# ArtoriasAbyssslayer/HashModNFFBanks-IDR

Measured on AMD Instinct MI355X. Metric: rays/sec fwd+bwd (hash+SDF MLP), higher is better.
Workload: dtype f32; 1 GPU; DTU-shaped synthetic uniform-sphere rays, MultiResHash L=16 T=2^19 F=2 (BASELINE.json configs[1]), full IDR training step (forward + IDRLoss + backward + clip + Adam), weights held at the geometric initialisation (lr = 0): the SURVEY.md 8(d) workload; grid_config=C2, rays_per_gpu=2048, global_rays=2048, parallelism=single GPU, world=1, ranks_seen=1, step=HIP-graph captured static-shape step

## Files before the change

hashmodnffbanks_idr_amd/csrc/hm_sdf.hip:

```cpp
#include "hm_common.h"

#include <math.h>
#include <stdlib.h>

namespace {

#include "hm_sdf_common.h"
#include "hm_trace_dev.h"

#ifdef HM_SDF_PHASE_PROBE
__device__ unsigned long long hm_probe_ts[128];
#define HM_PROBE(i_)                                                                                  \
    do {                                                                                              \
        if (blockIdx.x == 0 && threadIdx.x == 0 && it == 1 && (i_) < 120) hm_probe_ts[(i_)] = wall_clock64(); \
        if (blockIdx.x == 0 && threadIdx.x == 0 && it == 1 && ((i_) == 0 || (i_) == 100))                 \
            hm_probe_ts[120 + ((i_) != 0)] = clock64();         \
    } while (0)
#define HM_PROBE_WAVES(base_)                                                                                  \
    do {                                                                                                       \
        if (blockIdx.x == 0 && (threadIdx.x & 63) == 0 && it == 1 && li == 2) hm_probe_ts[(base_) + (threadIdx.x >> 6)] = wall_clock64(); \
    } while (0)
#define HM_PROBE_S(i_)                                                                                \
    do {                                                                                              \
        if (blockIdx.x == 0 && threadIdx.x == 0 && (i_) < 120) hm_probe_ts[(i_)] = wall_clock64();   \
// ... 361 lines not shown
        else if (n_loc <= 8 && !body16)
            sdf_small_body<FRAC, Tile8<8>>(lv, net, xp, n_loc, table, Bf, vp, 1, 1, lds, 0, 1 << 30);
        else
            sdf_small_body<FRAC, Tile16>(lv, net, xp, n_loc, table, Bf, vp, 1, 1, lds, 0, 1 << 30);
        __syncthreads();
        if (tid == 0) ctl[0] = 0;
        __syncthreads();
        if (mine) march_advance_ray(a, ray, ctl, slot_base);
        __syncthreads();
    }
}

__global__ __launch_bounds__(kThreadsSdf, 2) void mfma_f32_stream_kernel(int iters, float *out) {
    f32x16 acc00 = {0}, acc01 = {0}, acc10 = {0}, acc11 = {0};
    float a0 = (float)(threadIdx.x & 63) * 1e-3f, a1 = a0 + 0.5f, b0 = 1.0f - a0, b1 = 0.25f + a0;
    for (int it = 0; it < iters; ++it) {
#pragma unroll
        for (int r = 0; r < 4; ++r) {
            acc00 = __builtin_amdgcn_mfma_f32_32x32x2f32(a0, b0, acc00, 0, 0, 0);
            acc01 = __builtin_amdgcn_mfma_f32_32x32x2f32(a0, b1, acc01, 0, 0, 0);
            acc10 = __builtin_amdgcn_mfma_f32_32x32x2f32(a1, b0, acc10, 0, 0, 0);
            acc11 = __builtin_amdgcn_mfma_f32_32x32x2f32(a1, b1, acc11, 0, 0, 0);
        }
    }
    out[(size_t)blockIdx.x * kThreadsSdf + threadIdx.x] = acc00[0] + acc01[5] + acc10[9] + acc11[15];
}

__device__ __attribute__((noinline)) void secant_step_ray(const TraceArgs &a, int64_t q, int last) {
    secant_advance_ray(a, q, last);
}

template <int FRAC>
__device__ __forceinline__ void secant_role(const HmLevels &lv, const SdfNet &net, const float *__restrict__ table,
                                            const float *__restrict__ Bf, const TraceArgs &a, int n_iters, int64_t n,
                                            int pts, float *lds) {
    const int64_t n_tiles = (n + pts - 1) / pts;
    for (int it = 0; it < n_iters; ++it) {
        if (pts == 4)
            sdf_small_body<FRAC, Tile8<4>>(lv, net, a.w.pts, n, table, Bf, a.w.vals, 1, 1, lds, blockIdx.x, gridDim.x);
        else if (pts == 8)
            sdf_small_body<FRAC, Tile8<8>>(lv, net, a.w.pts, n, table, Bf, a.w.vals, 1, 1, lds, blockIdx.x, gridDim.x);
        else
            sdf_small_body<FRAC, Tile16>(lv, net, a.w.pts, n, table, Bf, a.w.vals, 1, 1, lds, blockIdx.x, gridDim.x);
        __syncthreads();
        for (int64_t tile = blockIdx.x; tile < n_tiles; tile += gridDim.x) {
            const int64_t q = tile * pts + threadIdx.x;
            if ((int)threadIdx.x < pts && q < n) secant_step_ray(a, q, it == n_iters - 1 ? 1 : 0);
        }
        __syncthreads();
    }
}

template <int FRAC>
__global__ __launch_bounds__(kThreadsSdf, 1) void trace_secant_kernel(HmLevels lv, SdfNet net,
                                                                       const float *__restrict__ table,
                                                                       const float *__restrict__ Bf, TraceArgs a,
                                                                       int n_iters, int64_t m8_max, int64_t m4_max,
                                                                       int64_t scan_hide) {
    extern __shared__ __align__(16) float lds[];
    const int64_t n = a.w.cnt[C_NSEC];
    if (n <= 0) return;
    const bool as_scan = scan_hide > 0 && a.w.cnt[C_NSEL_PTS] >= scan_hide;
    const int pts = as_scan ? 16 : (n <= m4_max ? 4 : (n <= m8_max ? 8 : 16));
    secant_role<FRAC>(lv, net, table, Bf, a, n_iters, n, pts, lds);
}

template <int FRAC>
__global__ __launch_bounds__(kThreadsSdf, 2) void sdf_scan_secant_kernel(HmLevels lv, SdfNet net,
                                                                          const float *__restrict__ table,
                                                                          const float *__restrict__ Bf, TraceArgs a,
                                                                          int n_iters, int64_t m8_max, int64_t m4_max,
                                                                          const float *__restrict__ scan_x,
                                                                          float *__restrict__ scan_out, int c_scan,
                                                                          int64_t scan_cap, int64_t scan_min,
                                                                          int64_t scan_hide, int c_prev1, int grid1,
                                                                          int c_prev2, int grid2) {
    extern __shared__ __align__(16) float lds[];
    const int64_t n_scan = min((int64_t)max(a.w.cnt[c_scan], 0), scan_cap);
    const int64_t n_sec = a.w.cnt[C_NSEC];
    if (n_sec > 0 && n_iters > 0) {
        const int pts = a.w.cnt[C_NSEL_PTS] >= scan_hide ? 16 : (n_sec <= m4_max ? 4 : (n_sec <= m8_max ? 8 : 16));
        secant_role<FRAC>(lv, net, table, Bf, a, n_iters, n_sec, pts, lds);
    }
    if (n_scan < scan_min) return;
    const int64_t tb = (n_scan + kPts - 1) / kPts;
    int64_t done = c_prev1 >= 0 ? fill_quota(max(a.w.cnt[c_prev1], 0), grid1, tb, scan_min) : 0;
    if (c_prev2 >= 0) done += fill_quota(max(a.w.cnt[c_prev2], 0), grid2, tb - done, scan_min);
    const int64_t skip = done * kPts;
    if (skip >= n_scan) return;
    const SdfFill none = {nullptr, nullptr, 0, 0};
    sdf64_run<FRAC, true>(lv, net, scan_x + skip * 3, n_scan - skip, table, Bf, scan_out + skip, 1, 1, lds,
                          reinterpret_cast<unsigned *>(a.w.cnt + C_TILE_CURSOR), none);
}

template <int KIND, int FRAC>
__device__ __forceinline__ void split_scan_range(const HmLevels &lv, const SdfNet &net_split, const float *__restrict__ table,
                                                 const float *__restrict__ Bf, const TraceArgs &a, int64_t scan_off,
                                                 int64_t n_scan, int64_t first, int64_t quota, unsigned *cursor, float *lds) {
    __shared__ unsigned s_scan_tile;
    if (quota <= 0) return;
    for (;;) {
        __syncthreads();
        if (threadIdx.x == 0) s_scan_tile = atomicAdd(cursor, 1u);
        __syncthreads();
        const int64_t k = s_scan_tile;
        if (k >= quota) break;
        sdf_split_tile<KIND, FRAC>(lv, net_split, a.w.pts + scan_off * 3, n_scan, table, Bf, a.w.vals + scan_off, 1, lds,
                                   first + k);
    }
}

template <int KIND, int FRAC>
__global__ __launch_bounds__(kThreadsSdf, 2) void sdf_refine_scan_kernel(HmLevels lv, SdfNet net, SdfNet net_split,
                                                                          const float *__restrict__ table,
                                                                          const float *__restrict__ Bf, TraceArgs a,
                                                                          int c_ref1, int c_ref2, int which,
                                                                          int64_t scan_off, int64_t chain_tiles) {
    extern __shared__ __align__(16) float lds[];
    const int64_t n_ref1 = min((int64_t)max(a.w.cnt[c_ref1], 0), a.w.cap);
    const int64_t n_ref2 = which ? min((int64_t)max(a.w.cnt[c_ref2], 0), a.w.cap) : 0;
    const int64_t n_ref = which ? n_ref2 : n_ref1;
    const int64_t n_scan = min((int64_t)max(a.w.cnt[C_NSEL_PTS], 0), a.w.cap);
    if (n_ref > 0) {
        const SdfFill none = {nullptr, nullptr, 0, 0};
        sdf64_run<FRAC, true>(lv, net, a.w.ref_pts, n_ref, table, Bf, a.w.ref_vals, 1, 1, lds,
                              reinterpret_cast<unsigned *>(a.w.cnt + (which ? C_XREF2_CURSOR : C_XREF_CURSOR)), none);
    }
    const ScanPool p = scan_pool_quota(n_scan, n_ref1, n_ref2, c_ref2 >= 0, gridDim.x, a.w.cnt[C_NSAMP], chain_tiles);
    split_scan_range<KIND, FRAC>(lv, net_split, table, Bf, a, scan_off, n_scan, which ? p.first[1] : p.first[0],
                                 which ? p.quota[1] : p.quota[0],
                                 reinterpret_cast<unsigned *>(a.w.cnt + (which ? C_XSCAN2_CURSOR : C_XSCAN_CURSOR)), lds);
}

template <int KIND, int FRAC>
__global__ __launch_bounds__(kThreadsSdf, 2) void sdf_split_scan_secant_kernel(HmLevels lv, SdfNet net, SdfNet net_split,
                                                                                const float *__restrict__ table,
                                                                                const float *__restrict__ Bf, TraceArgs a,
                                                                                int n_iters, int64_t m8_max, int64_t m4_max,
                                                                                int64_t scan_hide, int c_ref1, int c_ref2,
                                                                                int grid_x, int64_t scan_off,
                                                                                int64_t chain_tiles) {
    extern __shared__ __align__(16) float lds[];
    const int64_t n_sec = a.w.cnt[C_NSEC];
    if (n_sec > 0 && n_iters > 0) {
        const int pts = a.w.cnt[C_NSEL_PTS] >= scan_hide ? 16 : (n_sec <= m4_max ? 4 : (n_sec <= m8_max ? 8 : 16));
        secant_role<FRAC>(lv, net, table, Bf, a, n_iters, n_sec, pts, lds);
    }
    const int64_t n_scan = min((int64_t)max(a.w.cnt[C_NSEL_PTS], 0), a.w.cap);
    const int64_t n_ref1 = min((int64_t)max(a.w.cnt[c_ref1], 0), a.w.cap);
    const int64_t n_ref2 = c_ref2 >= 0 ? min((int64_t)max(a.w.cnt[c_ref2], 0), a.w.cap) : 0;
    const ScanPool p = scan_pool_quota(n_scan, n_ref1, n_ref2, c_ref2 >= 0, grid_x, a.w.cnt[C_NSAMP], chain_tiles);
    split_scan_range<KIND, FRAC>(lv, net_split, table, Bf, a, scan_off, n_scan, p.first[2], p.quota[2],
                                 reinterpret_cast<unsigned *>(a.w.cnt + C_YSCAN_CURSOR), lds);
}

static int sdf_net_fp32(const char *who, const HmLevels &lv, const hm_mlp_desc *mlp, int64_t emb_stride, SdfImage img,
                        SdfNet &net, bool *all_m16 = nullptr) {
    return sdf_net_from_desc(who, mlp, lv.E, emb_stride, img, 1, (lv.E + 7) / 8 * 2, false, net, all_m16);
}

constexpr size_t kLds16Max = 96 * 1024, kLds64Max = 160 * 1024, kLdsTrace = 64;

static int sdf_fp32_fits(const hm_mlp_desc *mlp, int E) {
    HmLevels lv = {};
    lv.E = E;
    SdfNet net;
    bool have16 = true;
    const int rc = sdf_net_fp32("hm_sdf_net_fits", lv, mlp, 0, kImgM16Optional, net, &have16);
    if (rc != HM_OK) return rc;
    HM_CHECK_ARG(sdf_lds64(net).bytes() + kLdsTrace <= kLds64Max, "hm_sdf_net_fits: network does not fit the 160 KB LDS tile");
    HM_CHECK_ARG(!have16 || sdf_lds_small(net, E, kPts16).bytes() + kLdsTrace <= kLds16Max,
                 "hm_sdf_net_fits: network does not fit the 16-point LDS tile");
    return HM_OK;
}

struct SmallTiles {
    int64_t m8_max, m4_max;
};
static SmallTiles sdf_small_tiles(int tile_points) {
// ... 100 lines not shown
        HM_CHECK_LAUNCH("hm_trace_march_tail");
        return HM_OK;
    });
}

int hm_trace_secant_persistent(const hm_grid_desc *desc, const hm_mlp_desc *mlp, const float *table, const float *B_fourier,
                               int frac_mode, int tile_points, const void *trace_args, int n_iters, int scan_rule,
                               void *stream) {
    HM_CHECK_ARG(desc && mlp && table && B_fourier && trace_args, "hm_trace_secant_persistent: NULL argument");
    HM_CHECK_ARG(frac_mode == HM_FRAC_REFERENCE || frac_mode == HM_FRAC_TRILINEAR, "hm_trace_secant_persistent: bad frac_mode");
    HM_CHECK_ARG(tile_points == 0 || tile_points == 4 || tile_points == 8 || tile_points == 16,
                 "hm_trace_secant_persistent: tile_points must be 0, 4, 8 or 16");
    const TraceArgs &a = *static_cast<const TraceArgs *>(trace_args);
    SdfNet net;
    const int rc = sdf_net_fp32("hm_trace_secant_persistent", desc->lv, mlp, 0, kImgM16, net);
    if (rc != HM_OK) return rc;
    if (a.n == 0 || n_iters <= 0) return HM_OK;
    const size_t lds = sdf_lds_small(net, desc->lv.E, kPts16).bytes();
    HM_CHECK_ARG(lds <= kLds16Max, "hm_trace_secant_persistent: network does not fit the 16-point LDS tile");
    const SmallTiles t = sdf_small_tiles(tile_points);
    const unsigned grid = sdf_small_grid(a.n, t, 256);
    return hm_frac_dispatch(frac_mode, [&](auto frac) {
        constexpr auto kernel = trace_secant_kernel<decltype(frac)::value>;
        const int rc = hm_allow_dynamic_lds<kernel>(96 * 1024);
        if (rc != HM_OK) return rc;
        hipLaunchKernelGGL(kernel, dim3(grid), dim3(kThreadsSdf), lds, as_stream(stream), desc->lv, net, table, B_fourier,
                           a, n_iters, t.m8_max, t.m4_max, (int64_t)((scan_rule && tile_points == 0) ? kTraceScanHide : 0));
        HM_CHECK_LAUNCH("hm_trace_secant_persistent");
        return HM_OK;
    });
}

int hm_trace_scan_secant(const hm_grid_desc *desc, const hm_mlp_desc *mlp, const float *table, const float *B_fourier,
                         int frac_mode, const void *trace_args, int n_iters, const float *scan_x, float *scan_out,
                         int64_t scan_capacity, int c_scan, int small_front, int c_prev1, int grid1, int c_prev2, int grid2,
                         void *stream) {
    HM_CHECK_ARG(desc && mlp && table && B_fourier && trace_args, "hm_trace_scan_secant: NULL argument");
    HM_CHECK_ARG(frac_mode == HM_FRAC_REFERENCE || frac_mode == HM_FRAC_TRILINEAR, "hm_trace_scan_secant: bad frac_mode");
    HM_CHECK_ARG(c_scan >= 0 && c_scan < C_COUNT && scan_capacity >= 0, "hm_trace_scan_secant: bad scan counter / capacity");
    HM_CHECK_ARG(small_front || (grid1 <= 0 && grid2 <= 0), "hm_trace_scan_secant: a refinement list has no filler tiles");
    const TraceArgs &a = *static_cast<const TraceArgs *>(trace_args);
    SdfNet net;
    int rc = sdf_net_fp32("hm_trace_scan_secant", desc->lv, mlp, 0, kImgM16, net);
    if (rc != HM_OK) return rc;
    if (a.n == 0) return HM_OK;
    HM_CHECK_ARG(scan_x && scan_out, "hm_trace_scan_secant: NULL scan pointer");
    if (small_front) {
        rc = hm_sdf_fwd(desc, mlp, scan_x, scan_capacity, table, B_fourier, scan_out, 1, 1, frac_mode, -1, a.w.cnt + c_scan, 0,
                        stream);
        if (rc != HM_OK) return rc;
    }
    const size_t lds16 = sdf_lds_small(net, desc->lv.E, kPts16).bytes(), lds64 = sdf_lds64(net).bytes();
    HM_CHECK_ARG(lds16 <= kLds16Max && lds64 <= kLds64Max - kLdsTrace, "hm_trace_scan_secant: network does not fit the LDS tiles");
    const size_t lds = lds16 > lds64 ? lds16 : lds64;
    static_assert(kTraceScanHide == 3 * 256 * kPts, "kTraceScanHide counts rounds of 64-point tiles");
    const int64_t scan_hide = kTraceScanHide;
    const int p1 = grid1 > 0 ? c_prev1 : -1, p2 = grid2 > 0 ? c_prev2 : -1;
    const SmallTiles t = sdf_small_tiles(0);
    return hm_frac_dispatch(frac_mode, [&](auto frac) {
        constexpr auto kernel = sdf_scan_secant_kernel<decltype(frac)::value>;
        const int rc = hm_allow_dynamic_lds<kernel>(160 * 1024 - 64);
        if (rc != HM_OK) return rc;
        hipLaunchKernelGGL(kernel, dim3(256), dim3(kThreadsSdf), lds, as_stream(stream), desc->lv, net, table, B_fourier, a,
                           n_iters, t.m8_max, t.m4_max, scan_x, scan_out, c_scan, scan_capacity,
                           (int64_t)(small_front ? kSdfSmall + 1 : 1), scan_hide, p1, grid1, p2, grid2);
        HM_CHECK_LAUNCH("hm_trace_scan_secant");
        return HM_OK;
    });
}

int hm_trace_refine_scan(const hm_grid_desc *desc, const hm_mlp_desc *mlp, const float *table, const float *B_fourier,
                         int frac_mode, const void *trace_args, int c_ref1, int c_ref2, int which, int64_t scan_off,
                         int64_t scan_capacity, int64_t chain_tiles, void *stream) {
    HM_CHECK_ARG(desc && mlp && table && B_fourier && trace_args, "hm_trace_refine_scan: NULL argument");
    HM_CHECK_ARG(frac_mode == HM_FRAC_REFERENCE || frac_mode == HM_FRAC_TRILINEAR, "hm_trace_refine_scan: bad frac_mode");
    HM_CHECK_ARG(c_ref1 >= 0 && c_ref1 < C_COUNT && c_ref2 < C_COUNT, "hm_trace_refine_scan: bad list counter");
    HM_CHECK_ARG((which == 0 || which == 1) && (which == 0 || c_ref2 >= 0) && chain_tiles >= 0,
                 "hm_trace_refine_scan: bad launch index / chain capacity");
    const TraceArgs &a = *static_cast<const TraceArgs *>(trace_args);
    static_assert(sizeof(HmLevels) + 2 * sizeof(SdfNet) + sizeof(TraceArgs) + 64 <= 4096, "kernel arguments exceed 4 KB");
    SdfNet net, net_split;
    size_t lds_split = 0;
    int rc = sdf_net_fp32("hm_trace_refine_scan", desc->lv, mlp, 0, kImgM16, net);
    if (rc == HM_OK) rc = sdf_split_net("hm_trace_refine_scan", desc->lv.E, mlp, 0, net_split, &lds_split);
    if (rc != HM_OK) return rc;
    if (a.n == 0) return HM_OK;
    HM_CHECK_ARG(a.w.pts && a.w.vals && a.w.ref_pts && a.w.ref_vals && a.w.cnt, "hm_trace_refine_scan: NULL workspace pointer");
    HM_CHECK_ARG(scan_off >= 0 && scan_capacity >= 0 && scan_capacity <= a.w.cap, "hm_trace_refine_scan: bad scan region");
    if (which == 0) {
        rc = hm_sdf_fwd(desc, mlp, a.w.pts + scan_off * 3, scan_capacity, table, B_fourier, a.w.vals + scan_off, 1, 1,
                        frac_mode, -1, a.w.cnt + C_NSEL_PTS, 0, stream);
        if (rc != HM_OK) return rc;
    }
    const size_t lds64 = sdf_lds64(net).bytes();
    HM_CHECK_ARG(lds64 <= kLds64Max - kLdsTrace && lds_split <= kLds64Max - kLdsTrace,
                 "hm_trace_refine_scan: network does not fit the LDS tiles");
    const size_t lds = lds_split > lds64 ? lds_split : lds64;
    const unsigned grid = refine_scan_grid(a.w.cap);
    const auto launch = [&](auto kind, auto frac) {
        constexpr auto kernel = sdf_refine_scan_kernel<decltype(kind)::value, decltype(frac)::value>;
        const int rc = hm_allow_dynamic_lds<kernel>(160 * 1024 - 64);
        if (rc != HM_OK) return rc;
        hipLaunchKernelGGL(kernel, dim3(grid), dim3(kThreadsSdf), lds, as_stream(stream), desc->lv, net, net_split, table,
                           B_fourier, a, c_ref1, c_ref2, which, scan_off, chain_tiles);
        HM_CHECK_LAUNCH("hm_trace_refine_scan");
        return HM_OK;
    };
    return hm_frac_dispatch(frac_mode, [&](auto frac) {
        if (mlp->split_kind == HM_SPLIT_BF16X2) return launch(std::integral_constant<int, HM_SPLIT_BF16X2>{}, frac);
        return launch(std::integral_constant<int, HM_SPLIT_F16X2>{}, frac);
    });
}

int hm_trace_split_scan_secant(const hm_grid_desc *desc, const hm_mlp_desc *mlp, const float *table,
                               const float *B_fourier, int frac_mode, const void *trace_args, int n_iters, int c_ref1,
                               int c_ref2, int64_t scan_off, int64_t scan_capacity, int64_t chain_tiles, void *stream) {
    HM_CHECK_ARG(desc && mlp && table && B_fourier && trace_args, "hm_trace_split_scan_secant: NULL argument");
    HM_CHECK_ARG(frac_mode == HM_FRAC_REFERENCE || frac_mode == HM_FRAC_TRILINEAR,
                 "hm_trace_split_scan_secant: bad frac_mode");
    HM_CHECK_ARG(c_ref1 >= 0 && c_ref1 < C_COUNT && c_ref2 < C_COUNT && chain_tiles >= 0,
                 "hm_trace_split_scan_secant: bad list counter / chain capacity");
    const TraceArgs &a = *static_cast<const TraceArgs *>(trace_args);
    SdfNet net, net_split;
    size_t lds_split = 0;
    int rc = sdf_net_fp32("hm_trace_split_scan_secant", desc->lv, mlp, 0, kImgM16, net);
    if (rc == HM_OK) rc = sdf_split_net("hm_trace_split_scan_secant", desc->lv.E, mlp, 0, net_split, &lds_split);
    if (rc != HM_OK) return rc;
    if (a.n == 0) return HM_OK;
    HM_CHECK_ARG(a.w.pts && a.w.vals && a.w.cnt, "hm_trace_split_scan_secant: NULL workspace pointer");
    HM_CHECK_ARG(scan_off >= 0 && scan_capacity >= 0 && scan_capacity <= a.w.cap, "hm_trace_split_scan_secant: bad scan region");
    const size_t lds16 = sdf_lds_small(net, desc->lv.E, kPts16).bytes();
    HM_CHECK_ARG(lds16 <= kLds16Max && lds_split <= kLds64Max - kLdsTrace,
                 "hm_trace_split_scan_secant: network does not fit the LDS tiles");
    const size_t lds = lds16 > lds_split ? lds16 : lds_split;
    const int grid_x = (int)refine_scan_grid(a.w.cap);
    const SmallTiles t = sdf_small_tiles(0);
    const auto launch = [&](auto kind, auto frac) {
        constexpr auto kernel = sdf_split_scan_secant_kernel<decltype(kind)::value, decltype(frac)::value>;
        const int rc = hm_allow_dynamic_lds<kernel>(160 * 1024 - 64);
        if (rc != HM_OK) return rc;
        hipLaunchKernelGGL(kernel, dim3(256), dim3(kThreadsSdf), lds, as_stream(stream), desc->lv, net, net_split, table,
                           B_fourier, a, n_iters, t.m8_max, t.m4_max, (int64_t)kTraceScanHide, c_ref1, c_ref2, grid_x,
                           scan_off, chain_tiles);
        HM_CHECK_LAUNCH("hm_trace_split_scan_secant");
        return HM_OK;
    };
    return hm_frac_dispatch(frac_mode, [&](auto frac) {
        if (mlp->split_kind == HM_SPLIT_BF16X2) return launch(std::integral_constant<int, HM_SPLIT_BF16X2>{}, frac);
        return launch(std::integral_constant<int, HM_SPLIT_F16X2>{}, frac);
    });
}

int hm_trace_scan_pool_plan(int64_t n_scan, int64_t n_ref1, int64_t n_ref2, int two_x, int grid_x, int64_t n_sec_bound,
                            int n_iters, int64_t chain_tiles, int64_t *first, int64_t *quota) {
    HM_CHECK_ARG(n_scan >= 0 && n_ref1 >= 0 && n_ref2 >= 0 && grid_x >= 1 && grid_x <= 256 && n_sec_bound >= 0 &&
                     n_iters >= 0 && chain_tiles >= -1 && first && quota,
                 "hm_trace_scan_pool_plan: bad argument");
    const ScanPool p = scan_pool_quota(n_scan, n_ref1, n_ref2, two_x != 0, grid_x, n_sec_bound,
                                       trace_chain_tiles(n_iters, chain_tiles));
    for (int k = 0; k < 3; ++k) {
        first[k] = p.first[k];
        quota[k] = p.quota[k];
    }
    return HM_OK;
}

static int sdf_fwd_impl(const HmLevels &lv, const hm_mlp_desc *mlp, const float *x, int64_t emb_stride, int64_t n,
                        const float *table, const float *B_fourier, float *out, int64_t out_stride, int out_cols,
                        int frac_mode, int tile_points, const int32_t *n_dev, int max_workgroups, void *stream,
                        const SdfFillArgs *fill, int *grid64_out) {
    HM_CHECK_ARG(n >= 0, "hm_sdf_fwd: n < 0");
    HM_CHECK_ARG(frac_mode == HM_FRAC_REFERENCE || frac_mode == HM_FRAC_TRILINEAR, "hm_sdf_fwd: bad frac_mode");
    const bool quarter = tile_points == HM_SDF_TILE64_QUARTER;
    if (quarter) tile_points = 64;
    HM_CHECK_ARG(tile_points == 0 || tile_points == 4 || tile_points == 8 || tile_points == 16 || tile_points == 64 ||
// ... 95 lines not shown
```

hashmodnffbanks_idr_amd/csrc/hm_sdf_tile64.h:

```cpp
#pragma once
#ifndef HM_PROBE
#define HM_PROBE(i_) do { } while (0)
#define HM_PROBE_WAVES(base_) do { } while (0)
#endif

constexpr int kFracEmb = 2;

constexpr int kPts = 64;
constexpr int kThreadsSdf = 512;
constexpr int kWaves = 8;
constexpr int kGroupFloats = kPts * 4;
typedef float f32x4q __attribute__((ext_vector_type(4)));

__device__ __forceinline__ void lane32_swap(float &a, float &b) {
    const auto r = __builtin_amdgcn_permlane32_swap(__float_as_uint(a), __float_as_uint(b), false, false);
    a = __uint_as_float(r[0]);
    b = __uint_as_float(r[1]);
}

__host__ __device__ inline SdfLds sdf_lds64(const SdfNet &net) {
    return sdf_lds(kPts, 1, net.x_groups * kGroupFloats, 1, net.emb_groups * kGroupFloats, kWaves);
}

struct SdfFill {
// ... 13 lines not shown

__device__ __forceinline__ int64_t fill_quota(int64_t n_own, int64_t grid, int64_t avail, int64_t run_min) {
    if (n_own < run_min || grid <= 0) return 0;
    const int64_t ta = (n_own + 63) / 64;
    const int64_t pad = (grid - ta % grid) % grid;
    return (pad > 0 && avail >= pad) ? pad : 0;
}

template <int FRAC, bool DYN, bool QUARTER = false>
__device__ __forceinline__ void sdf64_run(const HmLevels &lv, const SdfNet &net, const float *__restrict__ x, int64_t n,
                                          const float *__restrict__ table, const float *__restrict__ Bf,
                                          float *__restrict__ out, int64_t out_stride, int out_cols, float *lds,
                                          unsigned *cursor, const SdfFill &fb) {
    __shared__ unsigned s_next_tile;
    const SdfLds at = sdf_lds64(net);
    float *X = lds;
    float *EMB = lds + at.emb;
    float *SX = lds + at.sx;
    float *RED = lds + at.red;

    const int tid = threadIdx.x;
    const int wave = __builtin_amdgcn_readfirstlane(tid >> 6);
    const int lane = tid & 63;
    const int j = lane & 31;
    const int h = lane >> 5;
    const int m = lane & 15;
    const int q = lane >> 4;
    const int E = lv.E;
    const int64_t G = gridDim.x;
    const int64_t TA = (n + kPts - 1) / kPts;
    const int64_t n_fill = DYN ? 0 : fill_quota(n, G, max((fb.n + kPts - 1) / kPts - fb.tile0, (int64_t)0), 0);
    const int64_t rounds = n_fill > 0 ? (TA + n_fill) / G : (n / kPts) / G;
    const int64_t rem_base = rounds * G * kPts;
    const bool qt = QUARTER && !DYN && n_fill == 0 && n <= G * 16;
    const int64_t rem_step = qt ? 16 : (n - rem_base <= G * 32) ? 32 : kPts;

    for (int64_t it = 0;; ++it) {
        int64_t itr = it, wg = blockIdx.x;
        if (DYN) {
            __syncthreads();
            if (tid == 0) s_next_tile = atomicAdd(cursor, 1u);
            __syncthreads();
            const int64_t u = s_next_tile;
            itr = u / G;
            wg = u - itr * G;
        }
        if (itr > rounds) break;
        int64_t base;
        int cnt;
        const float *__restrict__ xs = x;
        float *__restrict__ os = out;
        if (n_fill > 0) {
            if (itr == rounds) break;
            const int64_t v = itr * G + wg;
            if (v < TA) {
                base = v * kPts;
                cnt = (int)min((int64_t)kPts, n - base);
            } else {
                base = (fb.tile0 + (v - TA)) * kPts;
                cnt = (int)min((int64_t)kPts, fb.n - base);
                xs = fb.x;
                os = fb.out;
            }
        } else if (itr < rounds) {
            base = (itr * G + wg) * kPts;
            cnt = kPts;
        } else {
// ... 222 lines not shown
```

hashmodnffbanks_idr_amd/csrc/hm_trace.hip:

```cpp
#include "hm_common.h"

#include <stdlib.h>
#include <string.h>

extern "C" int hm_trace_march_tail(const hm_grid_desc *desc, const hm_mlp_desc *mlp, const float *table,
                                   const float *B_fourier, int frac_mode, int body16, const void *trace_args, int first,
                                   int rounds, void *stream);

extern "C" int hm_trace_secant_persistent(const hm_grid_desc *desc, const hm_mlp_desc *mlp, const float *table,
                                          const float *B_fourier, int frac_mode, int tile_points, const void *trace_args,
                                          int n_iters, int scan_rule, void *stream);

extern "C" int hm_trace_scan_secant(const hm_grid_desc *desc, const hm_mlp_desc *mlp, const float *table,
                                    const float *B_fourier, int frac_mode, const void *trace_args, int n_iters,
                                    const float *scan_x, float *scan_out, int64_t scan_capacity, int c_scan,
                                    int small_front, int c_prev1, int grid1, int c_prev2, int grid2, void *stream);

extern "C" int hm_trace_refine_scan(const hm_grid_desc *desc, const hm_mlp_desc *mlp, const float *table,
                                    const float *B_fourier, int frac_mode, const void *trace_args, int c_ref1, int c_ref2,
                                    int which, int64_t scan_off, int64_t scan_capacity, int64_t chain_tiles, void *stream);

extern "C" int hm_trace_split_scan_secant(const hm_grid_desc *desc, const hm_mlp_desc *mlp, const float *table,
                                          const float *B_fourier, int frac_mode, const void *trace_args, int n_iters,
                                          int c_ref1, int c_ref2, int64_t scan_off, int64_t scan_capacity,
                                          int64_t chain_tiles, void *stream);

extern "C" int hm_sdf_fwd_fill(const hm_grid_desc *desc, const hm_mlp_desc *mlp, const float *x, int64_t n,
                               const float *table, const float *B_fourier, float *out, int frac_mode, const int32_t *n_dev,
                               const float *x_fill, float *out_fill, const int32_t *n_fill_dev, const int32_t *prev_dev,
                               int prev_grid, int *grid64_out, void *stream);

namespace {

constexpr int kTB = 256;

#include "hm_trace_dev.h"

__global__ __launch_bounds__(kTB) void trace_init_kernel(TraceArgs a) {
    const int64_t i = (int64_t)blockIdx.x * kTB + threadIdx.x;
    if (i >= a.n) return;
    trace_init_ray(a, i, a.w.cnt + C_ROUND0, 0);
}

__global__ __launch_bounds__(kTB) void trace_advance_kernel(TraceArgs a, int round) {
    const int64_t i = (int64_t)blockIdx.x * kTB + threadIdx.x;
    if (i >= a.n) return;
    trace_advance_ray(a, i, a.w.cnt + C_ROUND0 + round, 0);
}

__global__ __launch_bounds__(kTB) void trace_finalize_kernel(TraceArgs a) {
    const int64_t i = (int64_t)blockIdx.x * kTB + threadIdx.x;
    if (i >= a.n) return;
    const TraceWs &w = a.w;
    if (w.stage[i] != ST_DONE) atomicAdd(w.cnt + C_UNFINISHED, 1);
    const float t_s = w.t_s[i], t_e = w.t_e[i];
    a.out_mask[i] = t_s < t_e;
    a.out_t[i] = t_s;
    float px = 0.0f, py = 0.0f, pz = 0.0f;
// ... 460 lines not shown
    a.w.slot_s = ip; a.w.slot_e = ip + n; a.w.list_samp = ip + 2 * n; a.w.list_sec = ip + 3 * n; a.w.list_sel = ip + 4 * n;
    a.w.tail_slot = ip + 5 * n;
    uint8_t *bp = reinterpret_cast<uint8_t *>(base + L.off_b);
    a.w.live_s = bp; a.w.live_e = bp + n; a.w.stage = bp + 2 * n; a.w.it = bp + 3 * n; a.w.k = bp + 4 * n;
    a.w.is_samp = bp + 5 * n;
    a.w.pts = reinterpret_cast<float *>(base + L.off_pts);
    a.w.vals = reinterpret_cast<float *>(base + L.off_vals);
    a.w.cnt = reinterpret_cast<int32_t *>(base + L.off_cnt);
    a.w.cap = L.cap;
    a.w.ref_pts = reinterpret_cast<float *>(base + L.off_ref);
    a.w.ref_vals = a.w.ref_pts + 3 * (size_t)L.cap;
    a.w.ref_slot = reinterpret_cast<int32_t *>(a.w.ref_vals + (size_t)L.cap);
    a.w.guard = reinterpret_cast<int32_t *>(base);
    a.cam = cam_loc; a.dirs = ray_dirs; a.obj = object_mask; a.t_sphere = t_sphere; a.hit = hit_mask;
    a.fracs = sampler_fracs; a.steps_u = steps_u;
    a.out_pts = out_points; a.out_mask = out_net_mask; a.out_t = out_dists;
    a.n = n_rays; a.rays_per_image = rays_per_image;
    a.thr = cfg->sdf_threshold;
    for (int k = 0; k < 4; ++k) a.back[k] = (float)((1.0 - cfg->line_search_step) / (double)(1 << k));
    a.ls_iters = cfg->line_step_iters; a.max_it = cfg->sphere_tracing_iters; a.n_steps = cfg->n_steps;
    a.n_secant = cfg->n_secant_steps; a.training = cfg->training;
    a.head = (cfg->sampler_head >= 1 && cfg->sampler_head + 1 < cfg->n_steps) ? cfg->sampler_head : 0;
    a.tail_off = L.cap;
    const char *e_ov = getenv("HM_TRACE_OVERLAP");
    const bool overlap_ok = !(e_ov && atoi(e_ov) == 0);
    const bool overlap_shape = overlap_ok && cfg->training && !nffb && tile_points == 0 && cfg->n_secant_steps > 0 &&
                               n_rays <= kSdfSmall;
    const bool overlap = overlap_shape && !cfg->coarse_bf16;
    const bool sel_own = overlap || (guard && overlap_shape);
    a.sel_off = sel_own ? 2 * L.cap : -1;
    const bool cosched = guard && overlap_shape && !(e_ov && atoi(e_ov) == 1);
    const bool pool = cosched && !(e_ov && atoi(e_ov) == 2);
    const char *e_ct = getenv("HM_TRACE_POOL_CHAIN_TILES");
    const int64_t chain_tiles = pool ? trace_chain_tiles(cfg->n_secant_steps, (e_ct && atoi(e_ct) >= 0) ? atoi(e_ct) : -1) : 0;
    const int c_ref2 = (pool && a.head > 0) ? (int)C_GUARD_N2 : -1;

    hm_zero_u32_async(a.w.cnt, C_COUNT, st);
    const unsigned g_rays = (unsigned)((n_rays + kTB - 1) / kTB);
    const unsigned g_samp = (unsigned)((n_rays * cfg->n_steps + kTB - 1) / kTB);
    const unsigned g_rows = (unsigned)((n_rays + kGuardRows - 1) / kGuardRows);

    float *emb_ws = reinterpret_cast<float *>(base + L.off_emb);
    auto sdf = [&](int64_t capacity, const int32_t *n_dev) -> int {
        if (nffb) {
            const int rc = hm_nffb_fwd(desc, nffb, a.w.pts, capacity, table, B_fourier, emb_ws, emb_width, frac_mode,
                                       n_dev, stream);
            if (rc != HM_OK) return rc;
            return hm_sdf_fwd_emb(mlp, emb_ws, emb_width, emb_width, capacity, a.w.vals, 1, 1, tile_points, n_dev, 0,
                                  stream);
        }
        return hm_sdf_fwd(desc, mlp, a.w.pts, capacity, table, B_fourier, a.w.vals, 1, 1, frac_mode, tile_points, n_dev,
                          0, stream);
    };
    auto coarse = [&](int64_t off, int64_t capacity, const int32_t *n_dev) -> int {
        const float *p = a.w.pts + off * 3;
        float *v = a.w.vals + off;
        const int64_t run_min = kSdfSmall + 1;
        int rc;
        if (!cfg->coarse_bf16) {
            if (nffb) {
                rc = hm_nffb_fwd(desc, nffb, p, capacity, table, B_fourier, emb_ws, emb_width, frac_mode, n_dev, stream);
                if (rc == HM_OK)
                    rc = hm_sdf_fwd_emb(mlp, emb_ws, emb_width, emb_width, capacity, v, 1, 1, tile_points, n_dev, 0, stream);
            } else {
                rc = hm_sdf_fwd(desc, mlp, p, capacity, table, B_fourier, v, 1, 1, frac_mode, tile_points, n_dev, 0, stream);
            }
// ... 100 lines not shown
                                   (int)C_GUARD_N1);
            rc = guard_refine((int)C_GUARD_N1);
            if (rc != HM_OK) return rc;
        }
    }
    if (cfg->training && !overlap && !cosched) hipLaunchKernelGGL(closest_reduce_kernel, dim3(g_rays), dim3(kTB), 0, st, a);
    if (a.head > 0) {
        hipLaunchKernelGGL(sampler_head_kernel, dim3(g_rays), dim3(kTB), 0, st, a);
        hipLaunchKernelGGL(sampler_tail_points_kernel, dim3(g_samp), dim3(kTB), 0, st, a);
        int rc = overlap ? hm_sdf_fwd_fill(desc, mlp, a.w.pts + a.tail_off * 3, n_rays * (cfg->n_steps - a.head - 1), table,
                                           B_fourier, a.w.vals + a.tail_off, frac_mode, a.w.cnt + C_TAIL_PTS,
                                           a.w.pts + a.sel_off * 3, a.w.vals + a.sel_off, a.w.cnt + C_NSEL_PTS,
                                           a.w.cnt + c_first, grid_p1, &grid_p2, stream)
                         : coarse(a.tail_off, n_rays * (cfg->n_steps - a.head - 1), a.w.cnt + C_TAIL_PTS);
        if (rc != HM_OK) return rc;
        if (guard) {
            guard_noise(a.tail_off, n_rays * (cfg->n_steps - a.head - 1), (int)C_TAIL_PTS);
            hipLaunchKernelGGL(guard_select_sampler_kernel, dim3(g_rows), dim3(kTB), 0, st, a, 2, (int)C_TAIL_PTS,
                               sel_own ? c_first : (int)C_BIG_PTS, guard_min, (int)C_GUARD_N2);
            if (c_ref2 >= 0) {
                rc = hm_trace_refine_scan(desc, mlp, table, B_fourier, frac_mode, &a, (int)C_GUARD_N1, c_ref2, 1, a.sel_off,
                                          n_rays * cfg->n_steps, chain_tiles, stream);
                guard_patch(c_ref2);
            } else {
                rc = guard_refine((int)C_GUARD_N2);
            }
            if (rc != HM_OK) return rc;
        }
    }
    hipLaunchKernelGGL(sampler_reduce_kernel, dim3(g_rays), dim3(kTB), 0, st, a);
    if (cfg->n_secant_steps > 0) {
        hipLaunchKernelGGL(secant_points_kernel, dim3(g_rays), dim3(kTB), 0, st, a);
        if (overlap) {
            const int rc = hm_trace_scan_secant(desc, mlp, table, B_fourier, frac_mode, &a, cfg->n_secant_steps,
                                                a.w.pts + a.sel_off * 3, a.w.vals + a.sel_off, n_rays * cfg->n_steps,
                                                (int)C_NSEL_PTS, 1, c_first, grid_p1, (int)C_TAIL_PTS, grid_p2, stream);
            if (rc != HM_OK) return rc;
            hipLaunchKernelGGL(closest_reduce_kernel, dim3(g_rays), dim3(kTB), 0, st, a);
        } else if (pool) {
            int rc = hm_trace_split_scan_secant(desc, mlp, table, B_fourier, frac_mode, &a, cfg->n_secant_steps,
                                                (int)C_GUARD_N1, c_ref2, a.sel_off, n_rays * cfg->n_steps, chain_tiles,
                                                stream);
            if (rc != HM_OK) return rc;
            guard_noise(a.sel_off, n_rays * cfg->n_steps, (int)C_NSEL_PTS);
            hipLaunchKernelGGL(guard_select_closest_kernel, dim3(g_rows), dim3(kTB), 0, st, a, (int)C_NSEL_PTS, guard_min,
                               (int)C_GUARD_NC);
            rc = guard_refine((int)C_GUARD_NC, true);
            if (rc != HM_OK) return rc;
            hipLaunchKernelGGL(closest_reduce_kernel, dim3(g_rays), dim3(kTB), 0, st, a);
        } else if (cosched) {
            guard_noise(a.sel_off, n_rays * cfg->n_steps, (int)C_NSEL_PTS);
            hipLaunchKernelGGL(guard_select_closest_kernel, dim3(g_rows), dim3(kTB), 0, st, a, (int)C_NSEL_PTS, guard_min,
                               (int)C_GUARD_NC);
            const int rc = hm_trace_scan_secant(desc, mlp, table, B_fourier, frac_mode, &a, cfg->n_secant_steps, a.w.ref_pts,
                                                a.w.ref_vals, L.cap, (int)C_GUARD_NC, 0, -1, 0, -1, 0, stream);
            if (rc != HM_OK) return rc;
            guard_patch((int)C_GUARD_NC);
            hipLaunchKernelGGL(closest_reduce_kernel, dim3(g_rays), dim3(kTB), 0, st, a);
        } else if (!nffb && (tile_points == 0 || tile_points == 4 || tile_points == 8 || tile_points == 16) &&
            (tile_points != 0 || n_rays <= kSdfSmall)) {
            const int rc = hm_trace_secant_persistent(desc, mlp, table, B_fourier, frac_mode, tile_points, &a,
                                                      cfg->n_secant_steps, sel_own ? 1 : 0, stream);
            if (rc != HM_OK) return rc;
        } else {
            for (int s = 0; s < cfg->n_secant_steps; ++s) {
                int rc = sdf(n_rays, a.w.cnt + C_NSEC);
                if (rc != HM_OK) return rc;
                hipLaunchKernelGGL(secant_advance_kernel, dim3(g_rays), dim3(kTB), 0, st, a,
                                   s == cfg->n_secant_steps - 1 ? 1 : 0);
            }
        }
    }
    hipLaunchKernelGGL(count_evals_kernel, dim3(1), dim3(64), 0, st, a.w.cnt, rounds + 1, cfg->n_secant_steps);
    if (stats_out) {
        hipLaunchKernelGGL(hm_copy_u32_kernel, dim3(1), dim3(64), 0, st, reinterpret_cast<uint32_t *>(stats_out),
                           reinterpret_cast<const uint32_t *>(a.w.cnt + C_NSAMP), 16);
    }
    HM_CHECK_LAUNCH("hm_trace_forward");
    return HM_OK;
}

}
```

hashmodnffbanks_idr_amd/csrc/hm_trace_dev.h:

```cpp
#pragma once

enum : int32_t {
    C_ROUND0 = 0,
    C_NSAMP = 64,
    C_NSAMP_PTS = 65,
    C_NSEC = 66,
    C_NSEL = 67,
    C_NSEL_PTS = 68,
    C_ANY_LIVE = 69,
    C_EVALS = 70,
    C_UNFINISHED = 71,
    C_BIG_PTS = 73,
    C_NONFINITE = 72,
    C_NSAMP2 = 74,
    C_HEAD_PTS = 75,
    C_TAIL_PTS = 76,
    C_TILE_CURSOR = 77,
    C_GUARD_REFINED = 78,
    C_GUARD_MAXDEV = 79,
    C_GUARD_N1 = 80,
    C_GUARD_N2 = 81,
    C_GUARD_NC = 82,
    C_XREF_CURSOR = 83,
    C_XSCAN_CURSOR = 84,
    C_XREF2_CURSOR = 85,
    C_XSCAN2_CURSOR = 86,
    C_YSCAN_CURSOR = 87,
    C_COUNT = 96
};

constexpr float kGuardTau = 1.52587890625e-05f;
constexpr float kGuardTrip = kGuardTau * 0.25f;
constexpr int32_t kGuardTripped = 0x47554152;

constexpr int64_t kTraceScanHide = 3 * 256 * 64;

constexpr int64_t kScanTilesPerSecantIterPermille = 875;
inline int64_t trace_chain_tiles(int n_iters, int64_t given) {
    if (n_iters <= 0) return 0;
    return given >= 0 ? given : n_iters * kScanTilesPerSecantIterPermille / 1000;
}

enum : uint8_t { ST_WAIT_FIRST = 1, ST_WAIT_MARCH = 2, ST_WAIT_LS = 3, ST_DONE = 4 };

struct TraceWs {
    float *t_s, *t_e, *t_min, *t_max, *cur_s, *cur_e, *nxt_s, *nxt_e;
    float *z_lo, *z_hi, *v_lo, *v_hi, *z;
    int32_t *slot_s, *slot_e, *list_samp, *list_sec, *list_sel;
    int32_t *tail_slot;
    uint8_t *live_s, *live_e, *stage, *it, *k, *is_samp;
    float *pts;
    float *vals;
    int32_t *cnt;
    int64_t cap;
    float *ref_pts;
    float *ref_vals;
    int32_t *ref_slot;
    int32_t *guard;
};

struct TraceArgs {
    TraceWs w;
    const float *cam;
    const float *dirs;
    const uint8_t *obj;
    const float *t_sphere;
    const uint8_t *hit;
    const float *fracs;
    const float *steps_u;
    float *out_pts;
    uint8_t *out_mask;
    float *out_t;
    int64_t n, rays_per_image;
    float thr;
// ... 137 lines not shown
```

Baseline: 320,500 rays/s.

## Split secant iterations so the last steps overlap the guard refinement scan

In the pooled path, the secant loop is split. The first n_secant_steps-2 iterations run in the split scan kernel. The final iterations run in a second scan_secant launch that also evaluates the guard refinement list, replacing the separate guard_refine call. The scan kernel gains a QUARTER template variant using 16-point tiles and a smaller grid for small refinement lists, and the dynamic-cursor path now allows quarter tiles. This aims to hide the refinement SDF evaluation behind the tail secant steps and cut tail imbalance, at the cost of an extra iteration-range parameter and another launch-ordering dependency.

Result: faster. 328,700 rays/s, median of 6 (+2.6%).

```diff
diff --git a/hashmodnffbanks_idr_amd/csrc/hm_sdf.hip b/hashmodnffbanks_idr_amd/csrc/hm_sdf.hip
--- a/hashmodnffbanks_idr_amd/csrc/hm_sdf.hip
+++ b/hashmodnffbanks_idr_amd/csrc/hm_sdf.hip
@@ -417,10 +417,10 @@
 
 template <int FRAC>
 __device__ __forceinline__ void secant_role(const HmLevels &lv, const SdfNet &net, const float *__restrict__ table,
-                                            const float *__restrict__ Bf, const TraceArgs &a, int n_iters, int64_t n,
-                                            int pts, float *lds) {
+                                            const float *__restrict__ Bf, const TraceArgs &a, int it_first, int it_count,
+                                            int it_total, int64_t n, int pts, float *lds) {
     const int64_t n_tiles = (n + pts - 1) / pts;
-    for (int it = 0; it < n_iters; ++it) {
+    for (int it = it_first; it < it_first + it_count; ++it) {
         if (pts == 4)
             sdf_small_body<FRAC, Tile8<4>>(lv, net, a.w.pts, n, table, Bf, a.w.vals, 1, 1, lds, blockIdx.x, gridDim.x);
         else if (pts == 8)
@@ -430,7 +430,7 @@
         __syncthreads();
         for (int64_t tile = blockIdx.x; tile < n_tiles; tile += gridDim.x) {
             const int64_t q = tile * pts + threadIdx.x;
-            if ((int)threadIdx.x < pts && q < n) secant_step_ray(a, q, it == n_iters - 1 ? 1 : 0);
+            if ((int)threadIdx.x < pts && q < n) secant_step_ray(a, q, it == it_total - 1 ? 1 : 0);
         }
         __syncthreads();
     }
@@ -447,14 +447,15 @@
     if (n <= 0) return;
     const bool as_scan = scan_hide > 0 && a.w.cnt[C_NSEL_PTS] >= scan_hide;
     const int pts = as_scan ? 16 : (n <= m4_max ? 4 : (n <= m8_max ? 8 : 16));
-    secant_role<FRAC>(lv, net, table, Bf, a, n_iters, n, pts, lds);
-}
-
-template <int FRAC>
+    secant_role<FRAC>(lv, net, table, Bf, a, 0, n_iters, n_iters, n, pts, lds);
+}
+
+template <int FRAC, bool QUARTER>
 __global__ __launch_bounds__(kThreadsSdf, 2) void sdf_scan_secant_kernel(HmLevels lv, SdfNet net,
                                                                           const float *__restrict__ table,
                                                                           const float *__restrict__ Bf, TraceArgs a,
-                                                                          int n_iters, int64_t m8_max, int64_t m4_max,
+                                                                          int it_first, int n_iters, int it_total,
+                                                                          int64_t m8_max, int64_t m4_max,
                                                                           const float *__restrict__ scan_x,
                                                                           float *__restrict__ scan_out, int c_scan,
                                                                           int64_t scan_cap, int64_t scan_min,
@@ -465,7 +466,7 @@
     const int64_t n_sec = a.w.cnt[C_NSEC];
     if (n_sec > 0 && n_iters > 0) {
         const int pts = a.w.cnt[C_NSEL_PTS] >= scan_hide ? 16 : (n_sec <= m4_max ? 4 : (n_sec <= m8_max ? 8 : 16));
-        secant_role<FRAC>(lv, net, table, Bf, a, n_iters, n_sec, pts, lds);
+        secant_role<FRAC>(lv, net, table, Bf, a, it_first, n_iters, it_total, n_sec, pts, lds);
     }
     if (n_scan < scan_min) return;
     const int64_t tb = (n_scan + kPts - 1) / kPts;
@@ -474,8 +475,8 @@
     const int64_t skip = done * kPts;
     if (skip >= n_scan) return;
     const SdfFill none = {nullptr, nullptr, 0, 0};
-    sdf64_run<FRAC, true>(lv, net, scan_x + skip * 3, n_scan - skip, table, Bf, scan_out + skip, 1, 1, lds,
-                          reinterpret_cast<unsigned *>(a.w.cnt + C_TILE_CURSOR), none);
+    sdf64_run<FRAC, true, QUARTER>(lv, net, scan_x + skip * 3, n_scan - skip, table, Bf, scan_out + skip, 1, 1, lds,
+                                   reinterpret_cast<unsigned *>(a.w.cnt + C_TILE_CURSOR), none);
 }
 
 template <int KIND, int FRAC>
@@ -521,7 +522,8 @@
 __global__ __launch_bounds__(kThreadsSdf, 2) void sdf_split_scan_secant_kernel(HmLevels lv, SdfNet net, SdfNet net_split,
                                                                                 const float *__restrict__ table,
                                                                                 const float *__restrict__ Bf, TraceArgs a,
-                                                                                int n_iters, int64_t m8_max, int64_t m4_max,
+                                                                                int it_first, int n_iters, int it_total,
+                                                                                int64_t m8_max, int64_t m4_max,
                                                                                 int64_t scan_hide, int c_ref1, int c_ref2,
                                                                                 int grid_x, int64_t scan_off,
                                                                                 int64_t chain_tiles) {
@@ -529,7 +531,7 @@
     const int64_t n_sec = a.w.cnt[C_NSEC];
     if (n_sec > 0 && n_iters > 0) {
         const int pts = a.w.cnt[C_NSEL_PTS] >= scan_hide ? 16 : (n_sec <= m4_max ? 4 : (n_sec <= m8_max ? 8 : 16));
-        secant_role<FRAC>(lv, net, table, Bf, a, n_iters, n_sec, pts, lds);
+        secant_role<FRAC>(lv, net, table, Bf, a, it_first, n_iters, it_total, n_sec, pts, lds);
     }
     const int64_t n_scan = min((int64_t)max(a.w.cnt[C_NSEL_PTS], 0), a.w.cap);
     const int64_t n_ref1 = min((int64_t)max(a.w.cnt[c_ref1], 0), a.w.cap);
@@ -696,10 +698,12 @@
 }
 
 int hm_trace_scan_secant(const hm_grid_desc *desc, const hm_mlp_desc *mlp, const float *table, const float *B_fourier,
-                         int frac_mode, const void *trace_args, int n_iters, const float *scan_x, float *scan_out,
-                         int64_t scan_capacity, int c_scan, int small_front, int c_prev1, int grid1, int c_prev2, int grid2,
-                         void *stream) {
+                         int frac_mode, const void *trace_args, int it_first, int n_iters, int it_total, int quarter,
+                         const float *scan_x, float *scan_out, int64_t scan_capacity, int c_scan, int small_front,
+                         int c_prev1, int grid1, int c_prev2, int grid2, void *stream) {
     HM_CHECK_ARG(desc && mlp && table && B_fourier && trace_args, "hm_trace_scan_secant: NULL argument");
+    HM_CHECK_ARG(it_first >= 0 && n_iters >= 0 && it_first + n_iters <= it_total, "hm_trace_scan_secant: bad iteration range");
+    HM_CHECK_ARG(!quarter || !small_front, "hm_trace_scan_secant: quarter tiles are a refinement list's");
     HM_CHECK_ARG(frac_mode == HM_FRAC_REFERENCE || frac_mode == HM_FRAC_TRILINEAR, "hm_trace_scan_secant: bad frac_mode");
     HM_CHECK_ARG(c_scan >= 0 && c_scan < C_COUNT && scan_capacity >= 0, "hm_trace_scan_secant: bad scan counter / capacity");
     HM_CHECK_ARG(small_front || (grid1 <= 0 && grid2 <= 0), "hm_trace_scan_secant: a refinement list has no filler tiles");
@@ -721,15 +725,20 @@
     const int64_t scan_hide = kTraceScanHide;
     const int p1 = grid1 > 0 ? c_prev1 : -1, p2 = grid2 > 0 ? c_prev2 : -1;
     const SmallTiles t = sdf_small_tiles(0);
-    return hm_frac_dispatch(frac_mode, [&](auto frac) {
-        constexpr auto kernel = sdf_scan_secant_kernel<decltype(frac)::value>;
+    const int64_t qtiles = (scan_capacity + 15) / 16;
+    const unsigned grid = quarter && qtiles < 256 ? (unsigned)(qtiles > 0 ? qtiles : 1) : 256u;
+    const auto launch = [&](auto frac, auto q) {
+        constexpr auto kernel = sdf_scan_secant_kernel<decltype(frac)::value, decltype(q)::value>;
         const int rc = hm_allow_dynamic_lds<kernel>(160 * 1024 - 64);
         if (rc != HM_OK) return rc;
-        hipLaunchKernelGGL(kernel, dim3(256), dim3(kThreadsSdf), lds, as_stream(stream), desc->lv, net, table, B_fourier, a,
-                           n_iters, t.m8_max, t.m4_max, scan_x, scan_out, c_scan, scan_capacity,
+        hipLaunchKernelGGL(kernel, dim3(grid), dim3(kThreadsSdf), lds, as_stream(stream), desc->lv, net, table, B_fourier, a,
+                           it_first, n_iters, it_total, t.m8_max, t.m4_max, scan_x, scan_out, c_scan, scan_capacity,
                            (int64_t)(small_front ? kSdfSmall + 1 : 1), scan_hide, p1, grid1, p2, grid2);
         HM_CHECK_LAUNCH("hm_trace_scan_secant");
         return HM_OK;
+    };
+    return hm_frac_dispatch(frac_mode, [&](auto frac) {
+        return quarter ? launch(frac, std::true_type{}) : launch(frac, std::false_type{});
     });
 }
 
@@ -777,9 +786,12 @@
 }
 
 int hm_trace_split_scan_secant(const hm_grid_desc *desc, const hm_mlp_desc *mlp, const float *table,
-                               const float *B_fourier, int frac_mode, const void *trace_args, int n_iters, int c_ref1,
-                               int c_ref2, int64_t scan_off, int64_t scan_capacity, int64_t chain_tiles, void *stream) {
+                               const float *B_fourier, int frac_mode, const void *trace_args, int it_first, int n_iters,
+                               int it_total, int c_ref1, int c_ref2, int64_t scan_off, int64_t scan_capacity,
+                               int64_t chain_tiles, void *stream) {
     HM_CHECK_ARG(desc && mlp && table && B_fourier && trace_args, "hm_trace_split_scan_secant: NULL argument");
+    HM_CHECK_ARG(it_first >= 0 && n_iters >= 0 && it_first + n_iters <= it_total,
+                 "hm_trace_split_scan_secant: bad iteration range");
     HM_CHECK_ARG(frac_mode == HM_FRAC_REFERENCE || frac_mode == HM_FRAC_TRILINEAR,
                  "hm_trace_split_scan_secant: bad frac_mode");
     HM_CHECK_ARG(c_ref1 >= 0 && c_ref1 < C_COUNT && c_ref2 < C_COUNT && chain_tiles >= 0,
@@ -804,7 +816,8 @@
         const int rc = hm_allow_dynamic_lds<kernel>(160 * 1024 - 64);
         if (rc != HM_OK) return rc;
         hipLaunchKernelGGL(kernel, dim3(256), dim3(kThreadsSdf), lds, as_stream(stream), desc->lv, net, net_split, table,
-                           B_fourier, a, n_iters, t.m8_max, t.m4_max, (int64_t)kTraceScanHide, c_ref1, c_ref2, grid_x,
+                           B_fourier, a, it_first, n_iters, it_total, t.m8_max, t.m4_max, (int64_t)kTraceScanHide, c_ref1,
+                           c_ref2, grid_x,
                            scan_off, chain_tiles);
         HM_CHECK_LAUNCH("hm_trace_split_scan_secant");
         return HM_OK;
diff --git a/hashmodnffbanks_idr_amd/csrc/hm_sdf_tile64.h b/hashmodnffbanks_idr_amd/csrc/hm_sdf_tile64.h
--- a/hashmodnffbanks_idr_amd/csrc/hm_sdf_tile64.h
+++ b/hashmodnffbanks_idr_amd/csrc/hm_sdf_tile64.h
@@ -69,7 +69,7 @@
     const int64_t n_fill = DYN ? 0 : fill_quota(n, G, max((fb.n + kPts - 1) / kPts - fb.tile0, (int64_t)0), 0);
     const int64_t rounds = n_fill > 0 ? (TA + n_fill) / G : (n / kPts) / G;
     const int64_t rem_base = rounds * G * kPts;
-    const bool qt = QUARTER && !DYN && n_fill == 0 && n <= G * 16;
+    const bool qt = QUARTER && n_fill == 0 && n <= G * 16;
     const int64_t rem_step = qt ? 16 : (n - rem_base <= G * 32) ? 32 : kPts;
 
     for (int64_t it = 0;; ++it) {
diff --git a/hashmodnffbanks_idr_amd/csrc/hm_trace.hip b/hashmodnffbanks_idr_amd/csrc/hm_trace.hip
--- a/hashmodnffbanks_idr_amd/csrc/hm_trace.hip
+++ b/hashmodnffbanks_idr_amd/csrc/hm_trace.hip
@@ -12,18 +12,19 @@
                                           int n_iters, int scan_rule, void *stream);
 
 extern "C" int hm_trace_scan_secant(const hm_grid_desc *desc, const hm_mlp_desc *mlp, const float *table,
-                                    const float *B_fourier, int frac_mode, const void *trace_args, int n_iters,
-                                    const float *scan_x, float *scan_out, int64_t scan_capacity, int c_scan,
-                                    int small_front, int c_prev1, int grid1, int c_prev2, int grid2, void *stream);
+                                    const float *B_fourier, int frac_mode, const void *trace_args, int it_first,
+                                    int n_iters, int it_total, int quarter, const float *scan_x, float *scan_out,
+                                    int64_t scan_capacity, int c_scan, int small_front, int c_prev1, int grid1,
+                                    int c_prev2, int grid2, void *stream);
 
 extern "C" int hm_trace_refine_scan(const hm_grid_desc *desc, const hm_mlp_desc *mlp, const float *table,
                                     const float *B_fourier, int frac_mode, const void *trace_args, int c_ref1, int c_ref2,
                                     int which, int64_t scan_off, int64_t scan_capacity, int64_t chain_tiles, void *stream);
 
 extern "C" int hm_trace_split_scan_secant(const hm_grid_desc *desc, const hm_mlp_desc *mlp, const float *table,
-                                          const float *B_fourier, int frac_mode, const void *trace_args, int n_iters,
-                                          int c_ref1, int c_ref2, int64_t scan_off, int64_t scan_capacity,
-                                          int64_t chain_tiles, void *stream);
+                                          const float *B_fourier, int frac_mode, const void *trace_args, int it_first,
+                                          int n_iters, int it_total, int c_ref1, int c_ref2, int64_t scan_off,
+                                          int64_t scan_capacity, int64_t chain_tiles, void *stream);
 
 extern "C" int hm_sdf_fwd_fill(const hm_grid_desc *desc, const hm_mlp_desc *mlp, const float *x, int64_t n,
                                const float *table, const float *B_fourier, float *out, int frac_mode, const int32_t *n_dev,
@@ -550,6 +551,9 @@
     const bool cosched = guard && overlap_shape && !(e_ov && atoi(e_ov) == 1);
     const bool pool = cosched && !(e_ov && atoi(e_ov) == 2);
     const char *e_ct = getenv("HM_TRACE_POOL_CHAIN_TILES");
+    const char *e_tl = getenv("HM_TRACE_CHAIN_TAIL");
+    const int tail_want = (e_tl && atoi(e_tl) >= 0) ? atoi(e_tl) : kTraceChainTail;
+    const int k_tail = (pool && tail_want > 0 && cfg->n_secant_steps > tail_want) ? tail_want : 0;
     const int64_t chain_tiles = pool ? trace_chain_tiles(cfg->n_secant_steps, (e_ct && atoi(e_ct) >= 0) ? atoi(e_ct) : -1) : 0;
     const int c_ref2 = (pool && a.head > 0) ? (int)C_GUARD_N2 : -1;
 
@@ -716,28 +720,35 @@
     if (cfg->n_secant_steps > 0) {
         hipLaunchKernelGGL(secant_points_kernel, dim3(g_rays), dim3(kTB), 0, st, a);
         if (overlap) {
-            const int rc = hm_trace_scan_secant(desc, mlp, table, B_fourier, frac_mode, &a, cfg->n_secant_steps,
-                                                a.w.pts + a.sel_off * 3, a.w.vals + a.sel_off, n_rays * cfg->n_steps,
+            const int rc = hm_trace_scan_secant(desc, mlp, table, B_fourier, frac_mode, &a, 0, cfg->n_secant_steps,
+                                                cfg->n_secant_steps, 0, a.w.pts + a.sel_off * 3, a.w.vals + a.sel_off, n_rays * cfg->n_steps,
                                                 (int)C_NSEL_PTS, 1, c_first, grid_p1, (int)C_TAIL_PTS, grid_p2, stream);
             if (rc != HM_OK) return rc;
             hipLaunchKernelGGL(closest_reduce_kernel, dim3(g_rays), dim3(kTB), 0, st, a);
         } else if (pool) {
-            int rc = hm_trace_split_scan_secant(desc, mlp, table, B_fourier, frac_mode, &a, cfg->n_secant_steps,
+            const int n_front = cfg->n_secant_steps - k_tail;
+            int rc = hm_trace_split_scan_secant(desc, mlp, table, B_fourier, frac_mode, &a, 0, n_front, cfg->n_secant_steps,
                                                 (int)C_GUARD_N1, c_ref2, a.sel_off, n_rays * cfg->n_steps, chain_tiles,
                                                 stream);
             if (rc != HM_OK) return rc;
             guard_noise(a.sel_off, n_rays * cfg->n_steps, (int)C_NSEL_PTS);
             hipLaunchKernelGGL(guard_select_closest_kernel, dim3(g_rows), dim3(kTB), 0, st, a, (int)C_NSEL_PTS, guard_min,
                                (int)C_GUARD_NC);
-            rc = guard_refine((int)C_GUARD_NC, true);
+            if (k_tail > 0) {
+                rc = hm_trace_scan_secant(desc, mlp, table, B_fourier, frac_mode, &a, n_front, k_tail, cfg->n_secant_steps, 1,
+                                          a.w.ref_pts, a.w.ref_vals, L.cap, (int)C_GUARD_NC, 0, -1, 0, -1, 0, stream);
+                if (rc == HM_OK) guard_patch((int)C_GUARD_NC);
+            } else {
+                rc = guard_refine((int)C_GUARD_NC, true);
+            }
             if (rc != HM_OK) return rc;
             hipLaunchKernelGGL(closest_reduce_kernel, dim3(g_rays), dim3(kTB), 0, st, a);
         } else if (cosched) {
             guard_noise(a.sel_off, n_rays * cfg->n_steps, (int)C_NSEL_PTS);
             hipLaunchKernelGGL(guard_select_closest_kernel, dim3(g_rows), dim3(kTB), 0, st, a, (int)C_NSEL_PTS, guard_min,
                                (int)C_GUARD_NC);
-            const int rc = hm_trace_scan_secant(desc, mlp, table, B_fourier, frac_mode, &a, cfg->n_secant_steps, a.w.ref_pts,
-                                                a.w.ref_vals, L.cap, (int)C_GUARD_NC, 0, -1, 0, -1, 0, stream);
+            const int rc = hm_trace_scan_secant(desc, mlp, table, B_fourier, frac_mode, &a, 0, cfg->n_secant_steps,
+                                                cfg->n_secant_steps, 0, a.w.ref_pts, a.w.ref_vals, L.cap, (int)C_GUARD_NC, 0, -1, 0, -1, 0, stream);
             if (rc != HM_OK) return rc;
             guard_patch((int)C_GUARD_NC);
             hipLaunchKernelGGL(closest_reduce_kernel, dim3(g_rays), dim3(kTB), 0, st, a);
diff --git a/hashmodnffbanks_idr_amd/csrc/hm_trace_dev.h b/hashmodnffbanks_idr_amd/csrc/hm_trace_dev.h
--- a/hashmodnffbanks_idr_amd/csrc/hm_trace_dev.h
+++ b/hashmodnffbanks_idr_amd/csrc/hm_trace_dev.h
@@ -40,6 +40,8 @@
     if (n_iters <= 0) return 0;
     return given >= 0 ? given : n_iters * kScanTilesPerSecantIterPermille / 1000;
 }
+
+constexpr int kTraceChainTail = 2;
 
 enum : uint8_t { ST_WAIT_FIRST = 1, ST_WAIT_MARCH = 2, ST_WAIT_LS = 3, ST_DONE = 4 };
 
```
